# huggingface/parler-tts

Hardware: NVIDIA H100
Metric: audio codec tokens/sec (all codebooks) (higher is better)
Workload: dtype bf16

## Files before the change

### parler_tts_b200/csrc/attn_core.cuh

```cuda
#pragma once
#include "common.cuh"
#include "kernels.h"
#include "ptx.cuh"

namespace ptts {

constexpr int ATT_THREADS = 128;
constexpr int ATT_WARPS = 4;
constexpr int HD = PTTS_HEAD_DIM;

template <typename Sync>
__device__ __forceinline__ float block_reduce(float v, float* sh, bool is_max, int tid, Sync sync) {
  const int warp = tid >> 5, lane = tid & 31;
  v = is_max ? warp_max(v) : warp_sum(v);
  sync();
  if (lane == 0) sh[warp] = v;
  sync();
  float r = sh[0];
#pragma unroll
  for (int w = 1; w < ATT_WARPS; w++) r = is_max ? fmaxf(r, sh[w]) : r + sh[w];
  return r;
}

template <typename T>
// ... 150 lines not shown
}

namespace ptts {

template <typename T> struct AttChunk { static constexpr int CH = 32; };
template <> struct AttChunk<float> { static constexpr int CH = 16; };

template <typename T, int CH = AttChunk<T>::CH>
__host__ __device__ constexpr int attn_decode_smem_per_warp() {
  return 2 * 2 * CH * HD * (int)sizeof(T) + (3 * HD) * (int)sizeof(float);
}

__host__ __device__ __forceinline__ int attn_decode_warp_chunks(int n_cached, int CH, int part, int nparts) {
  const int n_chunks_all = (n_cached + CH - 1) / CH;
  return (n_chunks_all > part) ? (n_chunks_all - part + nparts - 1) / nparts : 0;
}

template <typename T, int CH>
__device__ __forceinline__ void attn_decode_issue_chunk(const T* kc, const T* vc, int n_cached, int i, int part, int nparts, T* stage, uint64_t* bar_p, int lane) {
  const int t0 = (part + nparts * i) * CH;
  const int n = (n_cached - t0 < CH) ? (n_cached - t0) : CH;
  const uint32_t bar = smem_u32(bar_p);
  if (lane == 0) mbar_expect_tx(bar, (uint32_t)(2 * n * HD * sizeof(T)));
  __syncwarp();
  if (lane < 2) {
    const T* src = (lane == 0 ? kc : vc) + (size_t)t0 * HD;
    T* dst = stage + (lane == 0 ? 0 : CH * HD);
    asm volatile("cp.async.bulk.shared::cluster.global.mbarrier::complete_tx::bytes [%0], [%1], %2, [%3];"
                 ::"r"(smem_u32(dst)), "l"(src), "r"((uint32_t)(n * HD * sizeof(T))), "r"(bar) : "memory");
  }
}

template <typename T, int CH = AttChunk<T>::CH>
__device__ __forceinline__ void attention_decode_request(const AttnArgs& p, int b, int kvh, int pos, unsigned char* stage0, uint64_t* bars, int lane,
                                                         int part, int nparts) {
  const T* kc = reinterpret_cast<const T*>(p.kcache) + (size_t)b * p.kv_b_stride + (size_t)kvh * p.kv_h_stride;
  const T* vc = reinterpret_cast<const T*>(p.vcache) + (size_t)b * p.kv_b_stride + (size_t)kvh * p.kv_h_stride;
  const int n_cached = p.cross ? p.kv_len : pos;
  if (attn_decode_warp_chunks(n_cached, CH, part, nparts) > 0)
    attn_decode_issue_chunk<T, CH>(kc, vc, n_cached, 0, part, nparts, reinterpret_cast<T*>(stage0), &bars[0], lane);
}

template <typename T, int CH = AttChunk<T>::CH>
__device__ __forceinline__ void attention_decode_sweep(const AttnArgs& p, int b, int kvh, int pos, unsigned char* stage0, unsigned char* rest, uint64_t* bars,
                                                       int lane, uint32_t& parity, int part = 0, int nparts = 1, float* xch = nullptr,
                                                       int pair_bar = 0, bool pre_issued = false, long long* prof = nullptr) {
  constexpr int STAGE_ELEMS = CH * HD;
  T* const st0 = reinterpret_cast<T*>(stage0);
  const int st_step = (int)(reinterpret_cast<T*>(rest) - st0);
  float* qs = reinterpret_cast<float*>(rest + 2 * STAGE_ELEMS * sizeof(T));
  float* kn = qs + HD;
  float* vn = kn + HD;
  const T* __restrict__ rope_cos = reinterpret_cast<const T*>(p.rope_cos) + (size_t)pos * HD;
  const T* __restrict__ rope_sin = reinterpret_cast<const T*>(p.rope_sin) + (size_t)pos * HD;
  const int rep = p.nh / p.nkv;
  T* kc = reinterpret_cast<T*>(p.kcache) + (size_t)b * p.kv_b_stride + (size_t)kvh * p.kv_h_stride;
  T* vc = reinterpret_cast<T*>(p.vcache) + (size_t)b * p.kv_b_stride + (size_t)kvh * p.kv_h_stride;
  const int lo = lane, hi = lane + HD / 2;
  const int n_cached = p.cross ? p.kv_len : pos;
  const int n_chunks = attn_decode_warp_chunks(n_cached, CH, part, nparts);

  auto issue = [&](int i) {
    attn_decode_issue_chunk<T, CH>(kc, vc, n_cached, i, part, nparts, st0 + (i & 1) * st_step, &bars[i & 1], lane);
  };
  auto wait_stage = [&](int st) {
    const uint32_t bar = smem_u32(&bars[st]);
    const uint32_t par = (parity >> st) & 1u;
    uint32_t ok, spins = 0;
    do {
      ok = mbar_try_wait(bar, par);
      if (!ok && ++spins > (1u << 16)) { if (lane == 0) printf("ptts: attention KV mbarrier timeout (cta %d b %d kvh %d stage %d cross %d n_cached %d chunks %d par %u)\n", (int)blockIdx.x, b, kvh, st, p.cross, n_cached, n_chunks, parity); __trap(); }
    } while (!ok);
    parity ^= (1u << st);
  };

  __syncwarp();
  if (!pre_issued) {
    fence_proxy_async_smem();
    if (n_chunks > 0) issue(0);
    if (n_chunks > 1) issue(1);
  } else if (n_chunks > 1) {
    fence_proxy_async_smem();
    issue(1);
  }

  const T* q_first = reinterpret_cast<const T*>(p.q) + (size_t)b * p.ldq + p.q_col0 + (size_t)(kvh * rep) * HD;
  const float qf0 = DT<T>::to_f(q_first[lo]), qf1 = DT<T>::to_f(q_first[hi]);
  if (!p.cross && part == 0) {
    const T* ksrc = reinterpret_cast<const T*>(p.knew) + (size_t)b * p.ldkv + p.k_col0 + kvh * HD;
    const T* vsrc = reinterpret_cast<const T*>(p.vnew) + (size_t)b * p.ldkv + p.v_col0 + kvh * HD;
    float x0 = DT<T>::to_f(ksrc[lo]), x1 = DT<T>::to_f(ksrc[hi]);
    if (p.rope) {
      const float y0 = rope_elem<T>(x0, x1, lo, rope_cos, rope_sin);
      const float y1 = rope_elem<T>(x1, x0, hi, rope_cos, rope_sin);
      x0 = y0; x1 = y1;
    }
    const T v0 = vsrc[lo], v1 = vsrc[hi];
    kc[(size_t)pos * p.kv_t_stride + kv_swz(pos, lo)] = DT<T>::from_f(x0);
    kc[(size_t)pos * p.kv_t_stride + kv_swz(pos, hi)] = DT<T>::from_f(x1);
    vc[(size_t)pos * p.kv_t_stride + kv_swz(pos, lo)] = v0;
    vc[(size_t)pos * p.kv_t_stride + kv_swz(pos, hi)] = v1;
    kn[lo] = DT<T>::rnd(x0); kn[hi] = DT<T>::rnd(x1);
    vn[lo] = DT<T>::to_f(v0); vn[hi] = DT<T>::to_f(v1);
  }
  const int grp = lane >> 3, d0 = (lane & 7) * 8;
  const int* km = p.key_mask ? p.key_mask + (size_t)b * p.mask_ld : nullptr;

  for (int rr = 0; rr < rep; rr++) {
    const int h = kvh * rep + rr;
    {
      const T* qsrc = reinterpret_cast<const T*>(p.q) + (size_t)b * p.ldq + p.q_col0 + h * HD;
      float x0 = (rr == 0) ? qf0 : DT<T>::to_f(qsrc[lo]), x1 = (rr == 0) ? qf1 : DT<T>::to_f(qsrc[hi]);
      if (p.rope) {
        const float y0 = rope_elem<T>(x0, x1, lo, rope_cos, rope_sin);
// ... 49 lines not shown
#pragma unroll
      for (int u = 0; u < PER; u++) {
        const int r = u * 4 + grp, rc = r < n ? r : n - 1;
        const float pe = expf(sloc[u] - m_new);
        lsum += pe;
        const float pw = DT<T>::rnd(pe);
        float vf[8];
        load8(vb + rc * HD + kv_swz(rc, d0), vf);
#pragma unroll
        for (int e = 0; e < 8; e++) acc[e] = fmaf(pw, vf[e], acc[e]);
      }
      lsum += __shfl_xor_sync(0xffffffffu, lsum, 8);
      lsum += __shfl_xor_sync(0xffffffffu, lsum, 16);
      l_run += lsum;
      m_run = m_new;
    };
    auto mask_bits = [&](int t0) -> int {
      const int t = t0 + lane;
      return (km != nullptr && lane < CH && t < p.mask_len && t < n_cached) ? km[t] : 1;
    };

    if (rr > 0) {
      __syncwarp();
      fence_proxy_async_smem();
      if (n_chunks > 0) issue(0);
      if (n_chunks > 1) issue(1);
    }
    for (int c = 0; c < n_chunks; c++) {
      const int st = c & 1;
      const int t0 = (part + nparts * c) * CH;
      const int n = (n_cached - t0 < CH) ? (n_cached - t0) : CH;
      const int mk = mask_bits(t0);
      wait_stage(st);
      if (prof != nullptr && c == 0 && rr == 0 && lane == 0) prof[11] = clock64();
      const T* stg = st0 + st * st_step;
      process(stg, stg + STAGE_ELEMS, __ballot_sync(0xffffffffu, mk != 0), n);
      if (c + 2 < n_chunks) {
        __syncwarp();
        fence_proxy_async_smem();
        issue(c + 2);
      }
    }
    if (!p.cross && part == 0) {
      __syncwarp();
      float s = 0.f;
      if (grp == 0) {
#pragma unroll
        for (int e = 0; e < 8; e++) s = fmaf(qv[e], kn[d0 + e], s);
      }
      s += __shfl_xor_sync(0xffffffffu, s, 1);
      s += __shfl_xor_sync(0xffffffffu, s, 2);
      s += __shfl_xor_sync(0xffffffffu, s, 4);
      s = __shfl_sync(0xffffffffu, s, 0) * p.scale;
      if (km != nullptr && pos < p.mask_len && km[pos] == 0) s = -INFINITY;
      const float m_new = fmaxf(m_run, s);
      if (m_new != -INFINITY) {
        const float corr = (m_run == -INFINITY) ? 0.f : expf(m_run - m_new);
        const float pe = (s == -INFINITY) ? 0.f : expf(s - m_new);
        const float pw = DT<T>::rnd(pe);
        l_run = l_run * corr + pe;
#pragma unroll
        for (int e = 0; e < 8; e++) acc[e] = acc[e] * corr + ((grp == 0) ? pw * vn[d0 + e] : 0.f);
        m_run = m_new;
      }
    }
#pragma unroll
    for (int e = 0; e < 8; e++) {
// ... 340 lines not shown
```

### parler_tts_b200/csrc/ptx.cuh

```cuda
#pragma once
#include "common.cuh"

namespace ptts {

__device__ __forceinline__ uint32_t smem_u32(const void* p) { return (uint32_t)__cvta_generic_to_shared(p); }

template <uint32_t COUNT>
__device__ __forceinline__ void mbar_init(uint64_t* bar) {
  asm volatile("mbarrier.init.shared::cta.b64 [%0], %1;" ::"r"(smem_u32(bar)), "n"(COUNT));
}
__device__ __forceinline__ void mbar_expect_tx(uint32_t bar, uint32_t bytes) {
  asm volatile("mbarrier.arrive.expect_tx.shared::cta.b64 _, [%0], %1;" ::"r"(bar), "r"(bytes) : "memory");
}
__device__ __forceinline__ void mbar_expect_tx(uint64_t* bar, uint32_t bytes) { mbar_expect_tx(smem_u32(bar), bytes); }
__device__ __forceinline__ uint32_t mbar_try_wait(uint32_t bar, uint32_t parity) {
  uint32_t ok;
  asm volatile("{\n.reg .pred p;\nmbarrier.try_wait.parity.shared::cta.b64 p, [%1], %2;\nselp.u32 %0, 1, 0, p;\n}"
               : "=r"(ok) : "r"(bar), "r"(parity) : "memory");
  return ok;
}
__device__ __forceinline__ uint32_t mbar_try_wait(uint64_t* bar, uint32_t parity) { return mbar_try_wait(smem_u32(bar), parity); }
__device__ __forceinline__ uint32_t mbar_try_wait_cluster(uint64_t* bar, uint32_t parity) {
  uint32_t ok;
  asm volatile("{\n.reg .pred p;\nmbarrier.try_wait.parity.acquire.cluster.shared::cta.b64 p, [%1], %2;\nselp.u32 %0, 1, 0, p;\n}"
               : "=r"(ok) : "r"(smem_u32(bar)), "r"(parity) : "memory");
  return ok;
}

__device__ __forceinline__ void bulk_g2s(uint32_t dst, const void* src, uint32_t bytes, uint32_t bar) {
  asm volatile("cp.async.bulk.shared::cluster.global.mbarrier::complete_tx::bytes [%0], [%1], %2, [%3];"
               ::"r"(dst), "l"(src), "r"(bytes), "r"(bar) : "memory");
}
__device__ __forceinline__ void bulk_g2s(void* dst, const void* src, uint32_t bytes, uint64_t* bar) {
  bulk_g2s(smem_u32(dst), src, bytes, smem_u32(bar));
}
__device__ __forceinline__ uint64_t l2_evict_first_policy() {
  uint64_t pol;
  asm volatile("createpolicy.fractional.L2::evict_first.b64 %0, 1.0;" : "=l"(pol));
  return pol;
}
__device__ __forceinline__ void bulk_g2s_evict_first(uint32_t dst, const void* src, uint32_t bytes, uint32_t bar) {
  asm volatile("cp.async.bulk.shared::cluster.global.mbarrier::complete_tx::bytes.L2::cache_hint [%0], [%1], %2, [%3], %4;"
               ::"r"(dst), "l"(src), "r"(bytes), "r"(bar), "l"(l2_evict_first_policy()) : "memory");
}
__device__ __forceinline__ void bulk_g2s_evict_first(void* dst, const void* src, uint32_t bytes, uint64_t* bar) {
  bulk_g2s_evict_first(smem_u32(dst), src, bytes, smem_u32(bar));
}
// ... 70 lines not shown
```

### parler_tts_b200/csrc/step2.cu

```cuda
#include "attn_core.cuh"
#include "common.cuh"
#include "kernels.h"
#include "ln_stats.cuh"
#include "sample_core.cuh"
#include "ptx.cuh"
#include "step.h"
#include "step_common.cuh"
#include <type_traits>

namespace ptts {
namespace cl {

constexpr int C = 2;
constexpr int V = 8;
constexpr int THREADS = 256;
constexpr int ROWS = 32;
constexpr int HROWS = 8;
constexpr int ATT_SMEM = attn_decode_smem_per_warp<bf16>();
constexpr int PROF_STRIDE = 16;
constexpr int QMAX = 6;
constexpr int OFF_STATS = 256, OFF_PART = 512, OFF_RES = 2560, OFF_CVEC = 3584;
constexpr int HDR = 5632;
constexpr int WB_BYTES = 65536;
constexpr int R_OFF = HDR + 2 * WB_BYTES;
constexpr int R_BYTES = 92160;
constexpr int QKV_OFF = R_BYTES - 2048;
constexpr int SMEM_BYTES = R_OFF + R_BYTES;
static_assert(SMEM_BYTES + 1024 <= 227 * 1024, "cluster step kernel shared memory");
static_assert(ROWS * (1024 / 2 + 8) * 2 + V * (256 + ROWS * 34 * 4) <= R_BYTES, "fc1 plan");
static_assert(HROWS * (1024 / 2 + 8) * 2 + V * C * (32 + 4 * 96 * 4) <= QKV_OFF, "QKV plan");
constexpr int ATT_STAGE = 2 * 32 * HD * 2;
constexpr int ATT_REST = ATT_SMEM - ATT_STAGE;
constexpr int ATT_S0_QKV = 34 * 1024;
constexpr int ATT_S0_QC = QKV_OFF - V * ATT_STAGE;
constexpr int ATT_S0_WB = WB_BYTES - ATT_STAGE;
static_assert(HROWS * (1024 / 2 + 8) * 2 + V * C * (32 + 4 * 96 * 4) <= ATT_S0_QKV && ATT_S0_QKV + 6 * ATT_STAGE <= QKV_OFF, "attention plan: QKV stages in R");
static_assert(HROWS * (1024 / 2 + 8) * 2 + V * C * (32 + 4 * 32 * 4) <= ATT_S0_QC, "attention plan: q_cross stages in R");
static_assert(2 * ATT_REST <= ATT_S0_QC && 2 * ATT_REST <= ATT_S0_QKV && 6 * ATT_REST <= ATT_S0_WB, "attention plan: second stages");
static_assert(6 * 8 * (1024 / 2) * 2 <= ATT_S0_WB && 16384 + 4 * 128 * 4 <= ATT_S0_WB, "attention plan: QKV weight jobs, out-proj job + pair merge");
static_assert(ROWS * (4096 / 4 + 8) * 2 + V * (256 + ROWS * 8 * 4) <= R_BYTES, "fc2 plan");

__device__ __forceinline__ void mbar_wait(uint64_t* bar, uint32_t parity, int what) {
  uint32_t ok, spins = 0;
  do {
    ok = mbar_try_wait_cluster(bar, parity);
    if (!ok && ++spins > (1u << 22)) { printf("ptts: cluster step mbarrier timeout (cta %d, barrier kind %d)\n", (int)blockIdx.x, what); __trap(); }
  } while (!ok);
}
__device__ __forceinline__ void st_async(uint32_t dst_cluster_addr, float v, uint32_t bar_cluster_addr) {
  asm volatile("st.async.shared::cluster.mbarrier::complete_tx::bytes.b32 [%0], %1, [%2];"
               ::"r"(dst_cluster_addr), "r"(__float_as_uint(v)), "r"(bar_cluster_addr) : "memory");
}
__device__ __forceinline__ void st_async(uint32_t dst_cluster_addr, float2 v, uint32_t bar_cluster_addr) {
  asm volatile("st.async.shared::cluster.mbarrier::complete_tx::bytes.v2.f32 [%0], {%1, %2}, [%3];"
               ::"r"(dst_cluster_addr), "f"(v.x), "f"(v.y), "r"(bar_cluster_addr) : "memory");
}
__device__ __forceinline__ uint32_t mapa(uint32_t addr, uint32_t rank) { uint32_t r; asm volatile("mapa.shared::cluster.u32 %0, %1, %2;" : "=r"(r) : "r"(addr), "r"(rank)); return r; }
__device__ __forceinline__ uint32_t cluster_rank() { uint32_t r; asm volatile("mov.u32 %0, %%cluster_ctarank;" : "=r"(r)); return r; }
__device__ __forceinline__ void cluster_arrive() { asm volatile("barrier.cluster.arrive.release.aligned;" ::: "memory"); }
__device__ __forceinline__ void cluster_wait() { asm volatile("barrier.cluster.wait.acquire.aligned;" ::: "memory"); }
__device__ __forceinline__ void cluster_arrive_reuse() { asm volatile("barrier.cluster.arrive.relaxed.aligned;" ::: "memory"); }

__host__ __device__ __forceinline__ int kslice(int kt) { return (kt & 7) >> 2; }
__host__ __device__ __forceinline__ int klocal(int kt) { return ((kt >> 3) << 2) | (kt & 3); }
__host__ __device__ __forceinline__ int kglobal(int rank, int lk) { return ((lk >> 2) << 3) | (rank << 2) | (lk & 3); }

template <int QN, int MT, bool STATS, bool ACC = false>
__device__ __forceinline__ void mma_slice(float (&out)[2][6][4], RowStatFrag& rst, const bf16* xs, int apitch, const uint4* wb, int KT, int kt0,
                                          int kt_end, int lrow, int lcol) {
  float acc[MT][QN][4];
#pragma unroll
  for (int a = 0; a < MT; a++)
#pragma unroll
// ... 1 lines not shown
#pragma unroll
      for (int e = 0; e < 4; e++) acc[a][j][e] = ACC ? out[a][j][e] : 0.f;
  for (int kt = kt0; kt < kt_end; kt += 4) {
    uint32_t a[MT][2][4];
#pragma unroll
    for (int mt = 0; mt < MT; mt++)
#pragma unroll
      for (int j = 0; j < 2; j++) ldmatrix_x4(a[mt][j], xs + (size_t)(mt * 16 + lrow) * apitch + kt * 32 + j * 16 + lcol);
    if (STATS) {
#pragma unroll
      for (int mt = 0; mt < MT; mt++) { row_stat_mma(rst, mt, a[mt][0]); row_stat_mma(rst, mt, a[mt][1]); }
    }
#pragma unroll
    for (int j = 0; j < QN; j++) {
      const uint4 w = wb[((size_t)j * KT + kt) * 32];
#pragma unroll
      for (int mt = 0; mt < MT; mt++) {
        mma_bf16_16816(acc[mt][j], a[mt][0], w.x, w.y);
        mma_bf16_16816(acc[mt][j], a[mt][1], w.z, w.w);
      }
    }
  }
#pragma unroll
  for (int mt = 0; mt < MT; mt++)
#pragma unroll
    for (int j = 0; j < QN; j++)
#pragma unroll
      for (int e = 0; e < 4; e++) out[mt][j][e] = acc[mt][j][e];
}

enum { PH_QKV = 0, PH_O = 1, PH_QC = 2, PH_OC = 3, PH_FC1 = 4, PH_FC2 = 5 };
constexpr int JOBS_PER_LAYER = 9;
constexpr int QKV_JOBS = 4;

__device__ __forceinline__ bool weight_job(const StepParams& p, int j, int cta, int rank, const char*& src, uint32_t& bytes) {
  const int nl = JOBS_PER_LAYER * p.L;
  if (j < nl) {
    const int l = j / JOBS_PER_LAYER, jl = j - JOBS_PER_LAYER * l;
    const int ph = jl < QKV_JOBS ? 0 : jl - (QKV_JOBS - 1);
    const int64_t idx = (ph == PH_QKV || ph == PH_QC) ? (int64_t)(cta >> 3) * C + rank : (int64_t)cta;
    const int64_t sz = p.lay.cp_slice[ph];
    bytes = (uint32_t)(ph == PH_QKV ? sz / QKV_JOBS : sz);
    src = p.blob + p.lay.layer0 + p.lay.layer_stride * l + p.lay.cp[ph] + idx * sz + (ph == PH_QKV ? jl * (sz / QKV_JOBS) : 0);
    return true;
  }
  const int task = cta + (int)gridDim.x * (j - nl);
  const int ntasks = p.K * p.V / 32;
  if (task >= ntasks) return false;
  bytes = (uint32_t)(4 * p.H * 16);
  src = p.blob + p.lay.heads + (int64_t)task * bytes;
  return true;
}

template <int ITEMS>
__global__ void __launch_bounds__(THREADS, 1) decode_step_cluster_kernel(const __grid_constant__ StepParams p) {
  extern __shared__ __align__(128) unsigned char smem[];
  Ctrl* ctrl = p.sa.ctrl;
  if (p.prof != nullptr && blockIdx.x == 0 && threadIdx.x == 0) p.prof[(size_t)(6 * p.L + 2) * PROF_STRIDE + 3] = clock64();
  if (ctrl->active == 0) return;
  int cur_len = ctrl->cur_len;
  const unsigned gen = (unsigned)ctrl->launch_gen;
  int pos = p.P + cur_len - 1;
  const int tid = threadIdx.x, warp = tid >> 5, lane = tid & 31;
  const int H = p.H, F = p.F, B = p.B;
  const int rank = (int)cluster_rank(), peer = rank ^ 1;
  const int cta = (int)blockIdx.x;
  const int cluster = cta >> 1;
  const int head = cluster >> 2, rblk = cluster & 3;
  const int Ks = H / C, KsF = F / 4;
  const int pitch = Ks + 8, pitchF = KsF + 8;
  const int qe = F / p.nh / 64;
  const int dgrp = warp & 1, e4 = warp >> 1;

  uint64_t* abar = reinterpret_cast<uint64_t*>(smem);
  uint64_t* wbar = abar + 1;
  uint64_t* xbar = abar + 3;
  uint64_t* attbars = reinterpret_cast<uint64_t*>(smem + 128);
  float* stats = reinterpret_cast<float*>(smem + OFF_STATS);
  float* part = reinterpret_cast<float*>(smem + OFF_PART);
  float* res_s = reinterpret_cast<float*>(smem + OFF_RES);
  float* cvec = reinterpret_cast<float*>(smem + OFF_CVEC);
  unsigned char* Rg = smem + R_OFF;
  const uint32_t peer_xbar = mapa(smem_u32(xbar), (uint32_t)peer);
  uint32_t par_a = 0, par_w = 0, par_x = 0, att_parity = 0;

  if (tid == 0) {
    mbar_init<1>(abar); mbar_init<1>(&wbar[0]); mbar_init<1>(&wbar[1]); mbar_init<1>(xbar);
    asm volatile("fence.mbarrier_init.release.cluster;" ::: "memory");
  }
  attention_decode_init_warp(attbars + 2 * warp, lane);
  cluster_arrive(); cluster_wait();
  unsigned* const bar_ctr = p.bar + (gen & 1u);
  unsigned bar_target = 0u;
  if (cta == 0 && tid == 0) p.bar[(gen + 1u) & 1u] = 0u;

  const char* blob = p.blob;
  long long* const prof0 = (p.prof != nullptr && cta == 0) ? p.prof : nullptr;
  long long* prof = prof0;
  prof_mark(prof, 0);

  auto issue_weight_job = [&](int j) {
    const char* src; uint32_t bytes;
    if (!weight_job(p, j, cta, rank, src, bytes)) return;
    mbar_expect_tx(&wbar[j & 1], bytes);
    bulk_g2s_evict_first(smem + HDR + (j & 1) * WB_BYTES, src, bytes, &wbar[j & 1]);
  };
  __shared__ int s_next_active;
  const int n_steps = (p.do_sample_phase && p.n_steps > 1 && prof0 == nullptr) ? p.n_steps : 1;
  int unfinished_prev = 0;
#pragma unroll 1
  for (int it = 0; it < n_steps; it++) {
  pos = p.P + cur_len - 1;
  prof = prof0;
  cluster_arrive_reuse();
  if (tid == 0) { issue_weight_job(0); issue_weight_job(1); }

  bf16* const x_img = p.cl_x;
  bf16* const a_img = p.cl_attn;
  bf16* const h_img = p.cl_h;
  const int x_slice_elems = ROWS * pitch, h_slice_elems = ROWS * pitchF;
// ... 34 lines not shown

  const int att_row = HROWS * rblk + 4 * rank + (warp >> 1);
  const int att_slice = kslice(2 * head), att_col = klocal(2 * head) * 32;

#pragma unroll 1
  for (int ph = 0; ph < n_phases; ph++) {
    const int l = ph / 6, sub = ph - 6 * l;
    prof = prof0 ? prof0 + (size_t)(ph + 1) * PROF_STRIDE : nullptr;
    prof_mark(prof, 0);
    const char* lb = blob + p.lay.layer0 + p.lay.layer_stride * l;
    const bool rowpart = (sub == PH_QKV || sub == PH_QC);
    const bool has_ln = (sub == PH_QKV || sub == PH_QC || sub == PH_FC1);
    const int q = (sub == PH_QKV) ? 6 : (sub == PH_QC ? 2 : (sub == PH_FC1 ? qe : 1));
    const int Nc = 4 * q * 8;
    const int KT = (sub == PH_FC2 ? KsF : Ks) >> 5;
    const int apitch = (sub == PH_FC2) ? pitchF : pitch;
    const int act_bytes = (rowpart ? HROWS : ROWS) * apitch * 2;
    const int RS = (q == 1) ? 8 : 8 * q + 2;
    const int blk = rowpart ? 32 + 4 * 16 * q * 4 : 256 + ROWS * RS * 4;
    unsigned char* const recv = Rg + ((act_bytes + 127) & ~127);
    const uint32_t peer_recv = mapa(smem_u32(recv), (uint32_t)peer);
    const uint32_t xbytes = 4u * (rowpart ? V * 4 * 16 * q + V / 2 * 4 * 2 : V / C * (ROWS * 8 * q + (has_ln ? ROWS * 2 : 0)));
    auto put = [&](int d, uint32_t off, auto v) {
      if (d == rank) *reinterpret_cast<decltype(v)*>(recv + off) = v;
      else st_async(peer_recv + off, v, peer_xbar);
    };
    const int j0 = JOBS_PER_LAYER * l + (sub == 0 ? 0 : sub + QKV_JOBS - 1);
    if (tid == 0) mbar_expect_tx(xbar, xbytes);

    auto att_stage0 = [&]() -> unsigned char* {
      if (sub == PH_QC) return Rg + ATT_S0_QC + warp * ATT_STAGE;
      return warp < 6 ? Rg + ATT_S0_QKV + warp * ATT_STAGE : smem + HDR + (warp - 6) * WB_BYTES + ATT_S0_WB;
    };
    if (rowpart && att_row < B)
      attention_decode_request<bf16>(decode_attn_args(p, l, pos, sub == PH_QC), att_row, head, pos, att_stage0(), attbars + 2 * warp, lane, warp & 1, 2);

    float cv1 = 0.f, cv2 = 0.f;
    if (has_ln) {
      const float* c1; int ntot;
      if (sub == PH_QKV) { c1 = reinterpret_cast<const float*>(lb + p.lay.c_qkv); ntot = p.qkv_rows; }
      else if (sub == PH_QC) { c1 = reinterpret_cast<const float*>(lb + p.lay.c_qc); ntot = H; }
      else { c1 = reinterpret_cast<const float*>(lb + p.lay.c_fc1); ntot = F; }
      const int nown = rowpart ? Nc : 8 * q;
      if (tid < nown) {
        int n;
        if (sub == PH_QKV) n = (tid >> 6) * (p.nh * HD) + head * HD + (tid & 63);
        else if (sub == PH_QC) n = head * HD + tid;
        else n = cta * 8 * q + tid;
        cv1 = c1[n];
        cv2 = c1[ntot + n];
      }
    }

    auto wait_job = [&](int j) {
      mbar_wait(&wbar[j & 1], (par_w >> (j & 1)) & 1u, 1);
      par_w ^= 1u << (j & 1);
    };
    auto ring = [&](int j) { return reinterpret_cast<const uint4*>(smem + HDR + (j & 1) * WB_BYTES) + lane; };
    wait_job(j0);
    if (sub == PH_QKV) wait_job(j0 + 1);
    mbar_wait(abar, par_a, 0);
    par_a ^= 1u;
    prof_mark(prof, 1);
    float acc[2][QMAX][4];
    RowStatFrag rst;
    row_stat_zero(rst);
    {
      const bf16* xs = reinterpret_cast<const bf16*>(Rg);
      if (rowpart) {
        auto head_pass = [&](auto pass_tag) {
          constexpr int P = decltype(pass_tag)::value;
          const int u = 2 * P + dgrp;
          float t[2][QMAX][4];
          if (sub == PH_QKV) mma_slice<6, 1, P == 0>(t, rst, xs, apitch, ring(j0 + u), KT, e4, KT, lrow & 7, lcol);
          else mma_slice<2, 1, P == 0>(t, rst, xs, apitch, ring(j0) + (size_t)(2 * u) * KT * 32, KT, e4, KT, lrow & 7, lcol);
          const int d = g >> 2;
          const uint32_t slot = (uint32_t)((8 * rank + warp) * blk);
          if (P == 0) {
            cluster_wait();
            if (dgrp == 0) {
              const uint32_t so = slot + 8 * (g & 3);
              if (t4 == 0) put(d, so, rst.s1[0][0]);
              if (t4 == (g >> 1)) put(d, so + 4, (g & 1) ? rst.sq[0][0][1] : rst.sq[0][0][0]);
            }
          }
#pragma unroll
          for (int j = 0; j < QMAX; j++)
            if (j < q) put(d, slot + 32 + 4 * ((g & 3) * 16 * q + P * 8 * q + j * 8 + 2 * t4), make_float2(t[0][j][0], t[0][j][1]));
        };
        head_pass(std::integral_constant<int, 0>{});
        if (sub == PH_QKV) {
          prof_mark(prof, 8);
          __syncthreads();
          if (tid == 0) { issue_weight_job(j0 + 2); issue_weight_job(j0 + 3); }
          wait_job(j0 + 2);
          wait_job(j0 + 3);
          prof_mark(prof, 9);
        }
        head_pass(std::integral_constant<int, 1>{});
      } else if (sub == PH_FC2) {
        auto quarter = [&](auto qq_tag) {
          constexpr int QQ = decltype(qq_tag)::value;
          const uint4* wq = ring(j0) + (size_t)dgrp * 2 * KT * 32 + (size_t)QQ * KT * 32;
          mma_slice<1, 2, false, QQ == 1>(acc, rst, xs, apitch, wq, 2 * KT, (e4 - QQ * KT) & 3, KT, lrow, lcol);
        };
        quarter(std::integral_constant<int, 0>{});
        prof_mark(prof, 8);
        __syncthreads();
        if (tid == 0) request_slice(h_img + (size_t)(2 * rank + 1) * h_slice_elems, (uint32_t)(h_slice_elems * 2));
        mbar_wait(abar, par_a, 0);
        par_a ^= 1u;
        prof_mark(prof, 9);
        quarter(std::integral_constant<int, 1>{});
      } else {
        const uint4* wb = ring(j0) + (size_t)(dgrp * q) * KT * 32;
        if (sub == PH_FC1) {
          if (q == 4) mma_slice<4, 2, true>(acc, rst, xs, apitch, wb, KT, e4, KT, lrow, lcol);
          else if (q == 2) mma_slice<2, 2, true>(acc, rst, xs, apitch, wb, KT, e4, KT, lrow, lcol);
          else mma_slice<1, 2, true>(acc, rst, xs, apitch, wb, KT, e4, KT, lrow, lcol);
        } else mma_slice<1, 2, false>(acc, rst, xs, apitch, wb, KT, e4, KT, lrow, lcol);
      }
    }
    prof_mark(prof, 2);
    prof_mark(prof, 12);
    if (!rowpart) cluster_wait();
    prof_mark(prof, 13);
    if (!rowpart) {
      const uint32_t slot = (uint32_t)((4 * rank + e4) * blk);
#pragma unroll
      for (int mt = 0; mt < 2; mt++)
#pragma unroll
        for (int j = 0; j < QMAX; j++) {
// ... 76 lines not shown
          float S1 = 0.f, S2 = 0.f;
#pragma unroll
          for (int e = 0; e < V; e++) {
            const float2 x = *reinterpret_cast<const float2*>(recv + (size_t)(8 * (e >> 2) + 2 * (e & 3)) * blk + r4 * 8);
            S1 += x.x; S2 += x.y;
          }
          const float ln_mean = S1 / (float)H;
          const float ln_rstd = rsqrtf(fmaxf(S2 / (float)H - ln_mean * ln_mean, 0.f) + p.eps);
          float v = 0.f;
#pragma unroll
          for (int e = 0; e < V; e++)
            v += reinterpret_cast<const float*>(recv + (size_t)(8 * (e >> 2) + 2 * (e & 3) + (u & 1)) * blk + 32)[r4 * QCW + cw];
          v = ln_rstd * (v - ln_mean * cvec[col]) + cvec[256 + col];
          qkv_s[idx] = __float2bfloat16_rn(v);
        }
      };
      if (sub == PH_QKV) gather(std::integral_constant<int, 48>{}); else gather(std::integral_constant<int, 16>{});
      static_assert(HD == 64, "QKV: 2 x 2 units of 6 n-tiles (q|k|v of a head), q_cross: 2 x 2 units of 2 n-tiles");
    }
    prof_mark(prof, 4);
    __syncthreads();
    cluster_arrive_reuse();

    if (rowpart) {
      if (att_row < B) {
        AttnArgs att = decode_attn_args(p, l, pos, sub == PH_QC);
        const bf16* qkv_s = reinterpret_cast<const bf16*>(Rg + QKV_OFF);
        const int row_base = HROWS * rblk + 4 * rank;
        const bf16* qbase = qkv_s - (size_t)row_base * Nc - (size_t)head * HD;
        att.q = qbase; att.ldq = Nc;
        att.ldo = pitch;
        att.out = a_img + (size_t)att_slice * x_slice_elems + att_col - (size_t)head * HD;
        if (sub == PH_QKV) { att.knew = qbase; att.vnew = qbase; att.ldkv = Nc; att.k_col0 = HD; att.v_col0 = 2 * HD; }
        unsigned char* wb0 = smem + HDR;
        unsigned char* held = wb0 + ((sub == PH_QKV ? j0 + 1 : j0) & 1) * WB_BYTES;
        unsigned char* other = wb0 + ((sub == PH_QKV ? j0 : j0 + 1) & 1) * WB_BYTES;
        unsigned char* rest = warp < 2 ? Rg + (size_t)warp * ATT_REST : held + (size_t)(warp - 2) * ATT_REST;
        float* xr = reinterpret_cast<float*>(other + 16384) + (warp >> 1) * 128;
        prof_mark(prof, 10);
        attention_decode_sweep<bf16>(att, att_row, head, pos, att_stage0(), rest, attbars + 2 * warp, lane, att_parity, warp & 1, 2, xr, (warp >> 1) + 1,
                                     true, tid == 0 ? prof : nullptr);
      }
      prof_mark(prof, 5);
    }
    prof_mark(prof, 6);
    if (p.prof != nullptr && l == p.L / 2 && tid == 0) {
      unsigned long long ns;
      asm volatile("mov.u64 %0, %%globaltimer;" : "=l"(ns));
      p.prof[(size_t)(n_phases + 4) * PROF_STRIDE + sub * (int)gridDim.x + cta] = (long long)ns;
    }

    const bool last = (ph + 1 == n_phases);
    const bf16* nimg; uint32_t nbytes;
    if (last) { nimg = x_img; nbytes = (uint32_t)(C * x_slice_elems * 2); }
    else slice_of((sub + 1) % 6, nimg, nbytes);
    const int held_job = sub == PH_QKV ? j0 + QKV_JOBS + 1 : (sub == PH_QC || sub == PH_OC) ? j0 + 2 : -1;
    bar_target = grid_sync(bar_ctr, bar_target, ph, false, nullptr, [&]() {
      request_slice(nimg, nbytes);
      if (held_job >= 0) issue_weight_job(held_job);
    });
    prof_mark(prof, 7);
  }
  cluster_wait();

  prof = prof0 ? prof0 + (size_t)(n_phases + 1) * PROF_STRIDE : nullptr;
  prof_mark(prof, 0);
  {
    const int ntasks = p.K * p.V / 32;
    const float* c1 = reinterpret_cast<const float*>(blob + p.lay.c_heads);
    const float* c2 = c1 + p.K * p.V;
    mbar_wait(abar, par_a, 3);
    par_a ^= 1u;
    const bf16* xs = reinterpret_cast<const bf16*>(Rg);
    const int KTH = H >> 5;
// ... 198 lines not shown
```

### parler_tts_b200/csrc/wgmma.cuh

```cuda
#pragma once
#include <cuda.h>

#include "common.cuh"
#include "ptx.cuh"

namespace ptts {
namespace wg {

constexpr int M_TILE = 128;
constexpr int K_STAGE = 64;
constexpr int STAGES = 3;
constexpr int CONSUMER_WARPS = 8;
constexpr int PRODUCER_WARP = CONSUMER_WARPS;
constexpr int THREADS = 32 * (CONSUMER_WARPS + 1);
constexpr int A_BYTES = M_TILE * K_STAGE * 2;

template <int N> constexpr int STAGE_BYTES = (A_BYTES + N * K_STAGE * 2 + 1023) & ~1023;
template <int N> constexpr size_t smem_bytes(int extra) { return 1024 + (size_t)STAGES * STAGE_BYTES<N> + 128 + extra; }

__device__ __forceinline__ void mbar_arrive(uint64_t* b) { asm volatile("mbarrier.arrive.shared::cta.b64 _, [%0];" ::"r"(smem_u32(b)) : "memory"); }
__device__ __forceinline__ void mbar_wait(uint64_t* b, uint32_t parity) {
  uint32_t ok, spins = 0;
  do {
    ok = mbar_try_wait(b, parity);
    if (!ok && ++spins > (1u << 24)) __trap();
  } while (!ok);
}
__device__ __forceinline__ void tma_load_2d(void* dst, const CUtensorMap* map, int c0, int c1, uint64_t* bar) {
  asm volatile("cp.async.bulk.tensor.2d.shared::cluster.global.tile.mbarrier::complete_tx::bytes [%0], [%1, {%2, %3}], [%4];"
               ::"r"(smem_u32(dst)), "l"(map), "r"(c0), "r"(c1), "r"(smem_u32(bar)) : "memory");
}
__device__ __forceinline__ void tma_load_3d(void* dst, const CUtensorMap* map, int c0, int c1, int c2, uint64_t* bar) {
  asm volatile("cp.async.bulk.tensor.3d.shared::cluster.global.tile.mbarrier::complete_tx::bytes [%0], [%1, {%2, %3, %4}], [%5];"
               ::"r"(smem_u32(dst)), "l"(map), "r"(c0), "r"(c1), "r"(c2), "r"(smem_u32(bar)) : "memory");
}

__device__ __forceinline__ uint64_t desc_sw128(uint32_t addr) {
  return (uint64_t)((addr >> 4) & 0x3FFF) | ((uint64_t)1 << 16) | ((uint64_t)(1024 >> 4) << 32) | ((uint64_t)1 << 62);
}

__device__ __forceinline__ void mma_n32(float (&d)[16], uint64_t da, uint64_t db, int accumulate) {
  asm volatile("{\n.reg .pred p;\nsetp.ne.b32 p, %18, 0;\n"
               "wgmma.mma_async.sync.aligned.m64n32k16.f32.bf16.bf16 {%0,%1,%2,%3,%4,%5,%6,%7,%8,%9,%10,%11,%12,%13,%14,%15}, %16, %17, p, 1, 1, 0, 0;\n}"
               : "+f"(d[0]), "+f"(d[1]), "+f"(d[2]), "+f"(d[3]), "+f"(d[4]), "+f"(d[5]), "+f"(d[6]), "+f"(d[7]), "+f"(d[8]), "+f"(d[9]), "+f"(d[10]), "+f"(d[11]), "+f"(d[12]), "+f"(d[13]), "+f"(d[14]), "+f"(d[15])
               : "l"(da), "l"(db), "r"(accumulate));
}
__device__ __forceinline__ void mma_n64(float (&d)[32], uint64_t da, uint64_t db, int accumulate) {
  asm volatile("{\n.reg .pred p;\nsetp.ne.b32 p, %34, 0;\n"
               "wgmma.mma_async.sync.aligned.m64n64k16.f32.bf16.bf16 {%0,%1,%2,%3,%4,%5,%6,%7,%8,%9,%10,%11,%12,%13,%14,%15,%16,%17,%18,%19,%20,%21,%22,%23,%24,%25,%26,%27,%28,%29,%30,%31}, %32, %33, p, 1, 1, 0, 0;\n}"
               : "+f"(d[0]), "+f"(d[1]), "+f"(d[2]), "+f"(d[3]), "+f"(d[4]), "+f"(d[5]), "+f"(d[6]), "+f"(d[7]), "+f"(d[8]), "+f"(d[9]), "+f"(d[10]), "+f"(d[11]), "+f"(d[12]), "+f"(d[13]), "+f"(d[14]), "+f"(d[15]), "+f"(d[16]), "+f"(d[17]), "+f"(d[18]), "+f"(d[19]), "+f"(d[20]), "+f"(d[21]), "+f"(d[22]), "+f"(d[23]), "+f"(d[24]), "+f"(d[25]), "+f"(d[26]), "+f"(d[27]), "+f"(d[28]), "+f"(d[29]), "+f"(d[30]), "+f"(d[31])
               : "l"(da), "l"(db), "r"(accumulate));
}
__device__ __forceinline__ void mma_n96(float (&d)[48], uint64_t da, uint64_t db, int accumulate) {
// ... 79 lines not shown
```

Baseline: 251,800.

## Stream QKV second-pass weights in pieces and pre-issue second attention KV chunk

Replaces the block-wide barrier and whole-job weight loads before the second QKV head pass with per-group counting mbarriers. The weights arrive in three pieces on separate mbarriers, so the MMA can start on the first piece while the others are still loading. After the pass, warps 2+ wait on the consumer barrier and issue the second KV chunk of the attention early into the held buffer. This aims to overlap weight transfer with compute and hide attention KV latency, at the cost of more mbarriers, more complex buffer ownership, and extra profiling hooks.

```diff
diff --git a/parler_tts_b200/csrc/attn_core.cuh b/parler_tts_b200/csrc/attn_core.cuh
--- a/parler_tts_b200/csrc/attn_core.cuh
+++ b/parler_tts_b200/csrc/attn_core.cuh
@@ -206,19 +206,19 @@
 }
 
 template <typename T, int CH = AttChunk<T>::CH>
-__device__ __forceinline__ void attention_decode_request(const AttnArgs& p, int b, int kvh, int pos, unsigned char* stage0, uint64_t* bars, int lane,
-                                                         int part, int nparts) {
+__device__ __forceinline__ void attention_decode_request(const AttnArgs& p, int b, int kvh, int pos, unsigned char* stage, uint64_t* bars, int lane,
+                                                         int part, int nparts, int chunk = 0) {
   const T* kc = reinterpret_cast<const T*>(p.kcache) + (size_t)b * p.kv_b_stride + (size_t)kvh * p.kv_h_stride;
   const T* vc = reinterpret_cast<const T*>(p.vcache) + (size_t)b * p.kv_b_stride + (size_t)kvh * p.kv_h_stride;
   const int n_cached = p.cross ? p.kv_len : pos;
-  if (attn_decode_warp_chunks(n_cached, CH, part, nparts) > 0)
-    attn_decode_issue_chunk<T, CH>(kc, vc, n_cached, 0, part, nparts, reinterpret_cast<T*>(stage0), &bars[0], lane);
+  if (attn_decode_warp_chunks(n_cached, CH, part, nparts) > chunk)
+    attn_decode_issue_chunk<T, CH>(kc, vc, n_cached, chunk, part, nparts, reinterpret_cast<T*>(stage), &bars[chunk], lane);
 }
 
 template <typename T, int CH = AttChunk<T>::CH>
 __device__ __forceinline__ void attention_decode_sweep(const AttnArgs& p, int b, int kvh, int pos, unsigned char* stage0, unsigned char* rest, uint64_t* bars,
                                                        int lane, uint32_t& parity, int part = 0, int nparts = 1, float* xch = nullptr,
-                                                       int pair_bar = 0, bool pre_issued = false, long long* prof = nullptr) {
+                                                       int pair_bar = 0, int pre_issued = 0, long long* prof = nullptr) {
   constexpr int STAGE_ELEMS = CH * HD;
   T* const st0 = reinterpret_cast<T*>(stage0);
   const int st_step = (int)(reinterpret_cast<T*>(rest) - st0);
@@ -249,11 +249,11 @@
   };
 
   __syncwarp();
-  if (!pre_issued) {
+  if (pre_issued == 0) {
     fence_proxy_async_smem();
     if (n_chunks > 0) issue(0);
     if (n_chunks > 1) issue(1);
-  } else if (n_chunks > 1) {
+  } else if (pre_issued == 1 && n_chunks > 1) {
     fence_proxy_async_smem();
     issue(1);
   }
@@ -369,7 +369,7 @@
       const int n = (n_cached - t0 < CH) ? (n_cached - t0) : CH;
       const int mk = mask_bits(t0);
       wait_stage(st);
-      if (prof != nullptr && c == 0 && rr == 0 && lane == 0) prof[11] = clock64();
+      if (prof != nullptr && c < 2 && rr == 0 && lane == 0) prof[c] = clock64();
       const T* stg = st0 + st * st_step;
       process(stg, stg + STAGE_ELEMS, __ballot_sync(0xffffffffu, mk != 0), n);
       if (c + 2 < n_chunks) {
diff --git a/parler_tts_b200/csrc/ptx.cuh b/parler_tts_b200/csrc/ptx.cuh
--- a/parler_tts_b200/csrc/ptx.cuh
+++ b/parler_tts_b200/csrc/ptx.cuh
@@ -13,6 +13,7 @@
   asm volatile("mbarrier.arrive.expect_tx.shared::cta.b64 _, [%0], %1;" ::"r"(bar), "r"(bytes) : "memory");
 }
 __device__ __forceinline__ void mbar_expect_tx(uint64_t* bar, uint32_t bytes) { mbar_expect_tx(smem_u32(bar), bytes); }
+__device__ __forceinline__ void mbar_arrive(uint64_t* b) { asm volatile("mbarrier.arrive.shared::cta.b64 _, [%0];" ::"r"(smem_u32(b)) : "memory"); }
 __device__ __forceinline__ uint32_t mbar_try_wait(uint32_t bar, uint32_t parity) {
   uint32_t ok;
   asm volatile("{\n.reg .pred p;\nmbarrier.try_wait.parity.shared::cta.b64 p, [%1], %2;\nselp.u32 %0, 1, 0, p;\n}"
diff --git a/parler_tts_b200/csrc/step2.cu b/parler_tts_b200/csrc/step2.cu
--- a/parler_tts_b200/csrc/step2.cu
+++ b/parler_tts_b200/csrc/step2.cu
@@ -17,7 +17,7 @@
 constexpr int ROWS = 32;
 constexpr int HROWS = 8;
 constexpr int ATT_SMEM = attn_decode_smem_per_warp<bf16>();
-constexpr int PROF_STRIDE = 16;
+constexpr int PROF_STRIDE = 32;
 constexpr int QMAX = 6;
 constexpr int OFF_STATS = 256, OFF_PART = 512, OFF_RES = 2560, OFF_CVEC = 3584;
 constexpr int HDR = 5632;
@@ -37,8 +37,7 @@
 static_assert(HROWS * (1024 / 2 + 8) * 2 + V * C * (32 + 4 * 96 * 4) <= ATT_S0_QKV && ATT_S0_QKV + 6 * ATT_STAGE <= QKV_OFF, "attention plan: QKV stages in R");
 static_assert(HROWS * (1024 / 2 + 8) * 2 + V * C * (32 + 4 * 32 * 4) <= ATT_S0_QC, "attention plan: q_cross stages in R");
 static_assert(2 * ATT_REST <= ATT_S0_QC && 2 * ATT_REST <= ATT_S0_QKV && 6 * ATT_REST <= ATT_S0_WB, "attention plan: second stages");
-static_assert(6 * 8 * (1024 / 2) * 2 <= ATT_S0_WB && 16384 + 4 * 128 * 4 <= ATT_S0_WB, "attention plan: QKV weight jobs, out-proj job + pair merge");
-static_assert(ROWS * (4096 / 4 + 8) * 2 + V * (256 + ROWS * 8 * 4) <= R_BYTES, "fc2 plan");
+static_assert(6 * 8 * (1024 / 2) * 2 <= ATT_S0_WB && 16384 + 4 * 128 * 4 <= ATT_S0_WB, "attention plan: QKV weight jobs, out-proj job + pair merge");static_assert(ROWS * (4096 / 4 + 8) * 2 + V * (256 + ROWS * 8 * 4) <= R_BYTES, "fc2 plan");
 
 __device__ __forceinline__ void mbar_wait(uint64_t* bar, uint32_t parity, int what) {
   uint32_t ok, spins = 0;
@@ -106,6 +105,9 @@
 enum { PH_QKV = 0, PH_O = 1, PH_QC = 2, PH_OC = 3, PH_FC1 = 4, PH_FC2 = 5 };
 constexpr int JOBS_PER_LAYER = 9;
 constexpr int QKV_JOBS = 4;
+constexpr int QKV_PIECES = 3;
+static_assert(QKV_JOBS % 2 == 0, "attention plan: out-proj's job (j0 + 4) lands in the buffer of job j0, not in the held one (j0 + 1)");
+static_assert(6 % QKV_PIECES == 0, "QKV: whole n-tiles per piece");
 
 __device__ __forceinline__ bool weight_job(const StepParams& p, int j, int cta, int rank, const char*& src, uint32_t& bytes) {
   const int nl = JOBS_PER_LAYER * p.L;
@@ -149,6 +151,8 @@
   uint64_t* abar = reinterpret_cast<uint64_t*>(smem);
   uint64_t* wbar = abar + 1;
   uint64_t* xbar = abar + 3;
+  uint64_t* cbar = abar + 4;
+  uint64_t* pbar = abar + 6;
   uint64_t* attbars = reinterpret_cast<uint64_t*>(smem + 128);
   float* stats = reinterpret_cast<float*>(smem + OFF_STATS);
   float* part = reinterpret_cast<float*>(smem + OFF_PART);
@@ -156,10 +160,13 @@
   float* cvec = reinterpret_cast<float*>(smem + OFF_CVEC);
   unsigned char* Rg = smem + R_OFF;
   const uint32_t peer_xbar = mapa(smem_u32(xbar), (uint32_t)peer);
-  uint32_t par_a = 0, par_w = 0, par_x = 0, att_parity = 0;
+  uint32_t par_a = 0, par_w = 0, par_x = 0, par_q = 0, att_parity = 0;
+  static_assert(128 >= 8 * (6 + 2 * QKV_PIECES), "mbarriers in front of the attention's");
 
   if (tid == 0) {
     mbar_init<1>(abar); mbar_init<1>(&wbar[0]); mbar_init<1>(&wbar[1]); mbar_init<1>(xbar);
+    mbar_init<4>(&cbar[0]); mbar_init<4>(&cbar[1]);
+    for (int i = 0; i < 2 * QKV_PIECES; i++) mbar_init<1>(&pbar[i]);
     asm volatile("fence.mbarrier_init.release.cluster;" ::: "memory");
   }
   attention_decode_init_warp(attbars + 2 * warp, lane);
@@ -260,6 +267,10 @@
       if (sub == PH_QC) return Rg + ATT_S0_QC + warp * ATT_STAGE;
       return warp < 6 ? Rg + ATT_S0_QKV + warp * ATT_STAGE : smem + HDR + (warp - 6) * WB_BYTES + ATT_S0_WB;
     };
+    auto att_rest = [&]() -> unsigned char* {
+      unsigned char* held = smem + HDR + ((sub == PH_QKV ? j0 + 1 : j0) & 1) * WB_BYTES;
+      return warp < 2 ? Rg + (size_t)warp * ATT_REST : held + (size_t)(warp - 2) * ATT_REST;
+    };
     if (rowpart && att_row < B)
       attention_decode_request<bf16>(decode_attn_args(p, l, pos, sub == PH_QC), att_row, head, pos, att_stage0(), attbars + 2 * warp, lane, warp & 1, 2);
 
@@ -296,12 +307,48 @@
     {
       const bf16* xs = reinterpret_cast<const bf16*>(Rg);
       if (rowpart) {
+        auto issue_pieces = [&](int g) {
+          const char* src; uint32_t bytes;
+          weight_job(p, j0 + 2 + g, cta, rank, src, bytes);
+          const uint32_t piece = bytes / QKV_PIECES;
+          unsigned char* dst = smem + HDR + ((j0 + g) & 1) * WB_BYTES;
+          for (int s = 0; s < QKV_PIECES; s++) {
+            mbar_expect_tx(&pbar[QKV_PIECES * g + s], piece);
+            bulk_g2s_evict_first(dst + s * piece, src + s * piece, piece, &pbar[QKV_PIECES * g + s]);
+          }
+        };
         auto head_pass = [&](auto pass_tag) {
           constexpr int P = decltype(pass_tag)::value;
           const int u = 2 * P + dgrp;
           float t[2][QMAX][4];
-          if (sub == PH_QKV) mma_slice<6, 1, P == 0>(t, rst, xs, apitch, ring(j0 + u), KT, e4, KT, lrow & 7, lcol);
-          else mma_slice<2, 1, P == 0>(t, rst, xs, apitch, ring(j0) + (size_t)(2 * u) * KT * 32, KT, e4, KT, lrow & 7, lcol);
+          if (sub == PH_QKV) {
+            if (P == 0) {
+              mma_slice<6, 1, true>(t, rst, xs, apitch, ring(j0 + u), KT, e4, KT, lrow & 7, lcol);
+            } else {
+              constexpr int PN = 6 / QKV_PIECES;
+#pragma unroll
+              for (int s = 0; s < QKV_PIECES; s++) {
+                if (s > 0) prof_mark(prof, 14 + 2 * s);
+                mbar_wait(&pbar[QKV_PIECES * dgrp + s], par_q, 5);
+                prof_mark(prof, s == 0 ? 9 : 15 + 2 * s);
+                float ts[2][QMAX][4];
+                mma_slice<PN, 1, false>(ts, rst, xs, apitch, ring(j0 + u) + (size_t)(PN * s) * KT * 32, KT, e4, KT, lrow & 7, lcol);
+#pragma unroll
+                for (int j = 0; j < PN; j++)
+#pragma unroll
+                  for (int e = 0; e < 4; e++) t[0][PN * s + j][e] = ts[0][j][e];
+              }
+            }
+            __syncwarp();
+            if (lane == 0) mbar_arrive(&cbar[dgrp]);
+            if (P == 0 && warp == dgrp && lane == 0) {
+              mbar_wait(&cbar[dgrp], 0u, 6);
+              issue_pieces(dgrp);
+            }
+            __syncwarp();
+          } else {
+            mma_slice<2, 1, P == 0>(t, rst, xs, apitch, ring(j0) + (size_t)(2 * u) * KT * 32, KT, e4, KT, lrow & 7, lcol);
+          }
           const int d = g >> 2;
           const uint32_t slot = (uint32_t)((8 * rank + warp) * blk);
           if (P == 0) {
@@ -317,15 +364,16 @@
             if (j < q) put(d, slot + 32 + 4 * ((g & 3) * 16 * q + P * 8 * q + j * 8 + 2 * t4), make_float2(t[0][j][0], t[0][j][1]));
         };
         head_pass(std::integral_constant<int, 0>{});
+        prof_mark(prof, 8);
+        head_pass(std::integral_constant<int, 1>{});
         if (sub == PH_QKV) {
-          prof_mark(prof, 8);
-          __syncthreads();
-          if (tid == 0) { issue_weight_job(j0 + 2); issue_weight_job(j0 + 3); }
-          wait_job(j0 + 2);
-          wait_job(j0 + 3);
-          prof_mark(prof, 9);
-        }
-        head_pass(std::integral_constant<int, 1>{});
+          par_q ^= 1u;
+          if (warp >= 2 && att_row < B) {
+            mbar_wait(&cbar[1], 1u, 6);
+            if (prof != nullptr && tid == 64) prof[25] = clock64();
+            attention_decode_request<bf16>(decode_attn_args(p, l, pos, false), att_row, head, pos, att_rest(), attbars + 2 * warp, lane, warp & 1, 2, 1);
+          }
+        }
       } else if (sub == PH_FC2) {
         auto quarter = [&](auto qq_tag) {
           constexpr int QQ = decltype(qq_tag)::value;
@@ -468,14 +516,13 @@
         att.ldo = pitch;
         att.out = a_img + (size_t)att_slice * x_slice_elems + att_col - (size_t)head * HD;
         if (sub == PH_QKV) { att.knew = qbase; att.vnew = qbase; att.ldkv = Nc; att.k_col0 = HD; att.v_col0 = 2 * HD; }
-        unsigned char* wb0 = smem + HDR;
-        unsigned char* held = wb0 + ((sub == PH_QKV ? j0 + 1 : j0) & 1) * WB_BYTES;
-        unsigned char* other = wb0 + ((sub == PH_QKV ? j0 : j0 + 1) & 1) * WB_BYTES;
-        unsigned char* rest = warp < 2 ? Rg + (size_t)warp * ATT_REST : held + (size_t)(warp - 2) * ATT_REST;
+        unsigned char* other = smem + HDR + ((sub == PH_QKV ? j0 : j0 + 1) & 1) * WB_BYTES;
         float* xr = reinterpret_cast<float*>(other + 16384) + (warp >> 1) * 128;
         prof_mark(prof, 10);
-        attention_decode_sweep<bf16>(att, att_row, head, pos, att_stage0(), rest, attbars + 2 * warp, lane, att_parity, warp & 1, 2, xr, (warp >> 1) + 1,
-                                     true, tid == 0 ? prof : nullptr);
+        if (prof != nullptr && tid == 64) prof[20] = clock64();
+        long long* aprof = prof == nullptr ? nullptr : tid == 0 ? prof + 23 : warp == 2 ? prof + 21 : nullptr;
+        attention_decode_sweep<bf16>(att, att_row, head, pos, att_stage0(), att_rest(), attbars + 2 * warp, lane, att_parity, warp & 1, 2, xr,
+                                     (warp >> 1) + 1, sub == PH_QKV && warp >= 2 ? 2 : 1, aprof);
       }
       prof_mark(prof, 5);
     }
diff --git a/parler_tts_b200/csrc/wgmma.cuh b/parler_tts_b200/csrc/wgmma.cuh
--- a/parler_tts_b200/csrc/wgmma.cuh
+++ b/parler_tts_b200/csrc/wgmma.cuh
@@ -18,7 +18,6 @@
 template <int N> constexpr int STAGE_BYTES = (A_BYTES + N * K_STAGE * 2 + 1023) & ~1023;
 template <int N> constexpr size_t smem_bytes(int extra) { return 1024 + (size_t)STAGES * STAGE_BYTES<N> + 128 + extra; }
 
-__device__ __forceinline__ void mbar_arrive(uint64_t* b) { asm volatile("mbarrier.arrive.shared::cta.b64 _, [%0];" ::"r"(smem_u32(b)) : "memory"); }
 __device__ __forceinline__ void mbar_wait(uint64_t* b, uint32_t parity) {
   uint32_t ok, spins = 0;
   do {
```

Result: no change. 253,200, median of 6 (+0.6%).
